# zilliztech/knowhere

Measured on NVIDIA H100. Metric: queries/sec at recall@10>=0.95, 10Mx128 f32 IVF_PQ, higher is better.
Workload: dtype f32

## Files before the change

knowhere_b200/csrc/kb2_index.cuh:

```cuda
#pragma once
#include <algorithm>
#include <functional>
#include <memory>
#include <mutex>
#include <vector>

#include "kb2_build.cuh"
#include "kb2_comm.h"
#include "kb2_fourcc.h"
#include "kb2_gemm_tc.cuh"
#include "kb2_ivf.cuh"
#include "kb2_ivfpq_tc.cuh"
#include "kb2_ivfflat_tc.cuh"
#include "kb2_json.h"
#include "kb2_large_k.cuh"

namespace kb2 {

constexpr int kMaxK = 1024;
constexpr int kMaxSortEntries = 8192;
constexpr int kMaxLargeK = 16384;
constexpr int64_t kLargeKScratch = 1ll << 30;

struct Counters {
// ... 1236 lines not shown
            KB2_CUDA_CHECK(cudaEventRecord(ev_join, side_stream));
            KB2_CUDA_CHECK(cudaStreamWaitEvent(st, ev_join, 0));
            side_pending = false;
        }
        mark("plan");
        pqtc::Params tp{};
        tp.metric = metric;
        tp.nq = (int)nq;
        tp.nprobe = nprobe;
        tp.queries = sp.queries;
        tp.qb16 = (const __nv_bfloat16*)s_qb16.p;
        tp.qnorm = s_qnorm.p;
        tp.n_items = items.n_items;
        tp.ticket = items.ticket;
        tp.item_list = items.list;
        tp.item_q0 = items.q0;
        tp.item_nq = items.nq;
        tp.pair_q = s_pair_q.p;
        tp.pair_base = s_pair_base.p;
        tp.bound = s_bound.p;
        tp.k_need = k_base;
        tp.margin_coef = (metric == KB2_METRIC_L2 ? 2.f : 1.f) * pqtc::kErrCoef * tc_rmax;
        tp.rmax = (metric == KB2_METRIC_L2) ? tc_rowmax : 0.f;
        tp.list_off = list_off.p;
        tp.list_len = list_len.p;
        tp.codes = (const uint4*)codes.p;
        tp.codes_plain = (const uint4*)tc_codes_plain.p;
        tp.npad = npad;
        tp.t1 = t1.p;
        tp.pqc = pqc.p;
        tp.pqc16 = (const uint4*)tc_pqc16.p;
        tp.bitset = sp.bitset;
        tp.rows = rows.p;
        const int n_logs = 2 * num_sms();
        const SurvivorLogs logs = alloc_logs(n_logs, (uint32_t)std::clamp<int64_t>(nq * 1024 / n_logs, 16384, 1 << 19));
        tp.log = logs.log;
        tp.log_cnt = logs.cnt;
        tp.log_cap = logs.cap;
        tp.qflag = s_cand_cnt.p + nq;
        tp.counters = d_counter.p;
        if (timing) KB2_CUDA_CHECK(cudaEventRecord(ev2, st));
        with_metric(metric, [&](auto m) {
            constexpr int MM = decltype(m)::value;
            if (tc_geom_18())
                launch<pqtc::ivfpq_tc_filter_kernel<MM, 1, 8>>(num_sms(), pqtc::THREADS, pqtc::TcCfg<1, 8>::SMEM_BYTES, st, tp);
            else
                launch<pqtc::ivfpq_tc_filter_kernel<MM, 3, 2>>(num_sms(), pqtc::THREADS, pqtc::TcCfg<3, 2>::SMEM_BYTES, st, tp);
        });
        if (timing) KB2_CUDA_CHECK(cudaEventRecord(ev3, st));
        KB2_CUDA_CHECK(cudaGetLastError());
#ifdef KB2_FILTER_STALLS
        pqtc::filter_stalls_print_kernel<<<1, 1, 0, st>>>(num_sms());
#endif
        mark("tc_filter");
        lm::scatter_survivors_kernel<<<dim3(16, n_logs), 256, 0, st>>>(logs.log, logs.cnt, logs.cap, s_cand.p, s_cand_cnt.p, kTcCandCap,
                                                                       tp.qflag, d_counter.p);
        const float* eval_lut = (tc_geom_18() && !dist) ? s_lut.p : nullptr;
        with_metric(metric, [&](auto m) {
            constexpr int MM = decltype(m)::value;
            if (tc_geom_18())
                pqtc::exact_eval_kernel<MM, 1, 8><<<(unsigned)nq, 128, 0, st>>>(sp.queries, pqc.p, eval_lut, s_bound.p, (const uint4*)codes.p,
                                                                               npad, t1.p, sp.bitset, rows.p, s_cand.p, s_cand_cnt.p,
                                                                               kTcCandCap, tp.qflag, logs.cnt + n_logs, k_base);
            else
                pqtc::exact_eval_kernel<MM, 3, 2><<<(unsigned)nq, 128, 0, st>>>(sp.queries, pqc.p, eval_lut, s_bound.p, (const uint4*)codes.p,
                                                                               npad, t1.p, sp.bitset, rows.p, s_cand.p, s_cand_cnt.p,
                                                                               kTcCandCap, tp.qflag, logs.cnt + n_logs, k_base);
        });
// ... 687 lines not shown
```

knowhere_b200/csrc/kb2_ivfpq_tc.cuh:

```cuda
#pragma once
#include <cuda_bf16.h>

#include <type_traits>
#include <utility>

#include "kb2_gemm_tc.cuh"
#include "kb2_ivf.cuh"
#include "kb2_listmajor.cuh"

namespace kb2 {
namespace pqtc {

using lm::TM;
constexpr int NQT = 256;
constexpr int THREADS = 512;
constexpr int GROUP_THREADS = 128;
constexpr int MAXW = 80;
constexpr int META_BYTES = 3 * NQT * 4;
template <int G, int DSUB>
struct TcCfg {
    static constexpr int M = 16 * G;
    static constexpr int KD = M * DSUB;
    static_assert(KD % 16 == 0 && (DSUB == 2 || DSUB == 4 || DSUB == 8), "unsupported PQ geometry");
    static constexpr int XCHUNK = KD / 8;
    static constexpr int KSTEPS = KD / 16 + 1;
    static constexpr int CHUNKS = 2 * KSTEPS;
    static constexpr int GRP_BYTES = CHUNKS * 128;
    static constexpr int TAB_BYTES = M * 256 * DSUB * 2;
    static constexpr int A_BYTES = (TM / 8) * GRP_BYTES, B_BYTES = (NQT / 8) * GRP_BYTES;
    static constexpr int OFF_TAB = 0;
    static constexpr int OFF_A = TAB_BYTES;
    static constexpr int OFF_B = OFF_A + 2 * A_BYTES;
    static constexpr int OFF_META = OFF_B + B_BYTES;
    static constexpr int OFF_BAR = OFF_META + 2 * META_BYTES;
    static constexpr size_t SMEM_BYTES = OFF_BAR + 256 + 128 ;
    static_assert(SMEM_BYTES <= 227 * 1024, "filter kernel shared memory");
};
constexpr int KD = 128;
constexpr float kErrCoef = 0.0085f;
constexpr float kAccCoef = 4e-5f;

struct Params {
    int metric;
    int nq, nprobe;
    const float* queries;
    const __nv_bfloat16* qb16;
    const float* qnorm;
    const int32_t* n_items;
    int32_t* ticket;
    const int32_t* item_list;
    const int32_t* item_q0;
    const int32_t* item_nq;
    const int32_t* pair_q;
    const float* pair_base;
    const float* bound;
    int k_need;
    float margin_coef;
    float rmax;
    const int64_t* list_off;
    const int32_t* list_len;
    const uint4* codes;
    const uint4* codes_plain;
    int64_t npad;
    const float* t1;
    const float* pqc;
    const uint4* pqc16;
    const uint8_t* bitset;
    const int32_t* rows;
    uint4* log;
    uint32_t* log_cnt;
    uint32_t log_cap;
    uint32_t* qflag;
    unsigned long long* counters;
};

template <typename F, int... I>
__device__ __forceinline__ void
static_for_impl(F&& f, std::integer_sequence<int, I...>) {
    (f(std::integral_constant<int, I>{}), ...);
}
template <int N, typename F>
__device__ __forceinline__ void
static_for(F&& f) {
    static_for_impl(f, std::make_integer_sequence<int, N>{});
}
template <int C0_, int W_>
struct BlockCols {
    static constexpr int C0 = C0_, W = W_;
};
template <int LO, int HI, typename F>
__device__ __forceinline__ void
dispatch_range(int n, F&& f) {
    if constexpr (LO == HI) {
        f(std::integral_constant<int, LO>{});
    } else {
        constexpr int MID = (LO + HI) / 2;
        if (n <= MID) dispatch_range<LO, MID>(n, f);
        else dispatch_range<MID + 1, HI>(n, f);
    }
}

__device__ __forceinline__ void
bar_sync_epi() {
    asm volatile("bar.sync 1, 256;" ::: "memory");
}
__device__ __forceinline__ uint64_t
make_desc_ns(uint32_t smem_addr, uint32_t grp_bytes) {
    uint64_t d = 0;
    d |= (uint64_t)((smem_addr & 0x3FFFFu) >> 4);
    d |= (uint64_t)(128 >> 4) << 16;
    d |= (uint64_t)(grp_bytes >> 4) << 32;
    return d;
}

#ifdef KB2_FILTER_STALLS
#define KB2_STALL_BEGIN(v) const long long v = clock64()
#define KB2_STALL_END(slot, v) stall[slot] += clock64() - (v)
constexpr int kStallMaxCtas = 1024, kStallSlots = 8;
__device__ unsigned long long g_filter_stalls[kStallMaxCtas][2][2][kStallSlots];
__global__ void
filter_stalls_print_kernel(int ctas) {
    for (int b = 0; b < min(ctas, kStallMaxCtas); b++) {
        printf("KB2STALL cta=%d", b);
        for (int r = 0; r < 2; r++) {
            printf(r == 0 ? " dec=" : " cons=");
            for (int i = 0; i < kStallSlots; i++)
                printf(i ? ",%llu" : "%llu", g_filter_stalls[b][r][0][i] + g_filter_stalls[b][r][1][i]);
        }
        printf("\n");
    }
}
#else
#define KB2_STALL_BEGIN(v)
#define KB2_STALL_END(slot, v)
#endif

__device__ __forceinline__ void
split3_bf16(float x, uint32_t& hi, uint32_t& mid, uint32_t& lo) {
    const __nv_bfloat16 h = __float2bfloat16_rn(x);
    hi = (uint32_t)__bfloat16_as_ushort(h);
    if (!(fabsf(x) < INFINITY)) { mid = 0u; lo = 0u; return; }
    const float r1 = x - __bfloat162float(h);
    const __nv_bfloat16 m = __float2bfloat16_rn(r1);
    const float r2 = r1 - __bfloat162float(m);
    mid = (uint32_t)__bfloat16_as_ushort(m);
    lo = (uint32_t)__bfloat16_as_ushort(__float2bfloat16_rn(r2));
}

template <int METRIC, int G, int DSUB>
__global__ void __launch_bounds__(THREADS, 1)
ivfpq_tc_filter_kernel(Params p) {
    using C = TcCfg<G, DSUB>;
    constexpr int KD = C::KD, XCHUNK = C::XCHUNK, KSTEPS = C::KSTEPS, GRP_BYTES = C::GRP_BYTES, TAB_BYTES = C::TAB_BYTES;
    constexpr int A_BYTES = C::A_BYTES, OFF_TAB = C::OFF_TAB, OFF_A = C::OFF_A, OFF_B = C::OFF_B, OFF_META = C::OFF_META,
                  OFF_BAR = C::OFF_BAR;
    extern __shared__ unsigned char smem_dyn[];
    const uint32_t raw = tc::smem_u32(smem_dyn);
    const uint32_t base = (raw + 127u) & ~127u;
    unsigned char* sm = smem_dyn + (base - raw);
    const uint32_t bars = base + OFF_BAR;
    auto bar_a_full = [&](int i) { return bars + 8u * i; };
    auto bar_a_empty = [&](int i) { return bars + 8u * (2 + i); };
    const uint32_t bar_b_full = bars + 8u * 8, bar_b_free = bars + 8u * 9;
    auto bar_meta_full = [&](int i) { return bars + 8u * (10 + i); };
    auto bar_meta_free = [&](int i) { return bars + 8u * (12 + i); };
    uint32_t* qcnt = (uint32_t*)(sm + OFF_BAR + 8 * 15);

    const int warp = __shfl_sync(0xffffffffu, (int)threadIdx.x >> 5, 0), lane = threadIdx.x & 31;
    const int n_items = *p.n_items;

    const lm::ItemRing<8> ring(sm + OFF_BAR + 144, p.ticket);
    ring.init();

    if (threadIdx.x == 0) {
        for (int i = 0; i < 2; i++) {
            tc::mbar_init(bar_a_full(i), GROUP_THREADS);
            tc::mbar_init(bar_a_empty(i), GROUP_THREADS);
            tc::mbar_init(bar_meta_full(i), 2 * GROUP_THREADS);
            tc::mbar_init(bar_meta_free(i), 2 * GROUP_THREADS);
        }
        tc::mbar_init(bar_b_full, 2 * GROUP_THREADS);
        tc::mbar_init(bar_b_free, 2 * GROUP_THREADS);
        qcnt[0] = qcnt[1] = qcnt[2] = qcnt[3] = 0;
        asm volatile("fence.mbarrier_init.release.cluster;" ::: "memory");
    }
#ifdef KB2_FILTER_STALLS
    long long stall[kStallSlots] = {0, 0, 0, 0, 0, 0, 0, 0};
    KB2_STALL_BEGIN(t_role);
#endif
    {
        uint4* tab = (uint4*)(sm + OFF_TAB);
        for (int i = threadIdx.x; i < TAB_BYTES / 16; i += THREADS) tab[i] = __ldg(p.pqc16 + i);
    }
    __syncthreads();
    const float inv_alpha = (METRIC == KB2_METRIC_L2) ? 0.5f : 1.f;

    if (warp < 8) {
        const int dt = threadIdx.x;
        const int dg = dt >> 7;
        const int tid = dt & 127;
        const uint4* tab = (const uint4*)(sm + OFF_TAB);
        auto write_meta = [&](int item, int it) {
            KB2_STALL_BEGIN(t_meta);
            const int par = it & 1;
            tc::mbar_wait(bar_meta_free(par), (((uint32_t)it >> 1) & 1u) ^ 1u);
            const int q0 = p.item_q0[item];
            const int nqi = p.item_nq[item];
            float* m_h = (float*)(sm + OFF_META + par * META_BYTES);
            float* m_base = m_h + NQT;
            int* m_q = (int*)(m_base + NQT);
            const int j = dt;
            float h = -INFINITY, bs = 0.f;
            int q = -1;
            if (j < nqi) {
                q = p.pair_q[q0 + j];
                bs = p.pair_base[q0 + j];
                const float bnd = p.bound[q];
                if (!(bnd < INFINITY)) {
                    p.qflag[q] = 1u;
                    if (p.counters) atomicAdd(p.counters + 6, 1ull << 32);
                } else {
                    const float margin = p.margin_coef * p.qnorm[q] * 1.01f + 1e-30f;
                    const float h0 = (bnd + margin - bs) * inv_alpha;
                    h = h0 + kAccCoef * (fabsf(h0) + p.rmax) + 1e-30f;
                }
            }
            m_h[j] = h;
            m_base[j] = bs;
            m_q[j] = q;
            tc::mbar_arrive(bar_meta_full(par));
            KB2_STALL_END(5, t_meta);
        };
        uint32_t g0 = 0;
        int it = 0;
        int item = ring.at_warp(0);
        if (item < n_items) write_meta(item, 0);
        for (; item < n_items; it++) {
            const int item_next = ring.at_warp(it + 1);
            const int l = p.item_list[item];
            const int nqi = p.item_nq[item];
            const int nmma = (nqi + 15) & ~15;
            const int len = p.list_len[l];
            const int64_t off = p.list_off[l];
            const int ntiles = (len + TM - 1) / TM;
            const int par = it & 1;
            const int t_first = (int)((dg - (int)(g0 & 1u)) & 1);
            uint4 w_next[G];
#pragma unroll
            for (int g = 0; g < G; g++) w_next[g] = make_uint4(0, 0, 0, 0);
            float t_next = 0.f;
            const uint4* code_src = (DSUB == 8) ? p.codes : p.codes_plain;
            if (t_first < ntiles && off + (int64_t)t_first * TM + tid < p.npad) {
#pragma unroll
                for (int g = 0; g < G; g++) w_next[g] = ldg_stream_u4(code_src + (int64_t)g * p.npad + off + (int64_t)t_first * TM + tid);
                if (METRIC == KB2_METRIC_L2) t_next = __ldg(p.t1 + off + (int64_t)t_first * TM + tid);
            }
            auto decode_tile = [&](int t) {
                KB2_STALL_BEGIN(t_dec);
                const uint32_t g = g0 + (uint32_t)t;
                uint4 w[G];
#pragma unroll
                for (int gg = 0; gg < G; gg++) w[gg] = w_next[gg];
                const float tv = t_next;
                {
                    const int64_t pn = off + (int64_t)(t + 2) * TM + tid;
                    if (t + 2 < ntiles && pn < p.npad) {
#pragma unroll
                        for (int gg = 0; gg < G; gg++) w_next[gg] = ldg_stream_u4(code_src + (int64_t)gg * p.npad + pn);
                        if (METRIC == KB2_METRIC_L2) t_next = __ldg(p.t1 + pn);
                    }
                }
                float r = INFINITY;
                if (t * TM + tid < len) r = (METRIC == KB2_METRIC_L2) ? 0.5f * tv : 0.f;
                uint32_t rh, rm, rl;
                split3_bf16(-r, rh, rm, rl);
                uint4 v[XCHUNK];
                if constexpr (DSUB == 8) {
#pragma unroll
                    for (int gg = 0; gg < G; gg++) {
                        const uint32_t ww[4] = {w[gg].x, w[gg].y, w[gg].z, w[gg].w};
#pragma unroll
                        for (int s = 0; s < 16; s++) {
                            const uint32_t byte = (ww[s >> 2] >> (8 * (s & 3))) & 255u;
                            v[gg * 16 + s] = tab[byte * (16 * G) + gg * 16 + ((s + tid) & 15)];
                        }
                    }
                } else {
                    constexpr int SPC = 8 / DSUB;
                    constexpr int WPS = DSUB / 2;
                    const uint32_t* tab32 = reinterpret_cast<const uint32_t*>(tab);
#pragma unroll
                    for (int c = 0; c < XCHUNK; c++) {
                        uint32_t u[4];
#pragma unroll
                        for (int j = 0; j < SPC; j++) {
                            const int m = c * SPC + j;
                            const uint4 wg = w[m >> 4];
                            const int b = m & 15;
                            const uint32_t word = (b < 4) ? wg.x : (b < 8) ? wg.y : (b < 12) ? wg.z : wg.w;
                            const uint32_t byte = (word >> (8 * (b & 3))) & 255u;
#pragma unroll
                            for (int x = 0; x < WPS; x++) u[j * WPS + x] = tab32[(m * 256 + byte) * WPS + x];
                        }
                        v[c] = make_uint4(u[0], u[1], u[2], u[3]);
                    }
                }
                KB2_STALL_BEGIN(t_ae);
                tc::mbar_wait(bar_a_empty(dg), ((g >> 1) & 1u) ^ 1u);
                KB2_STALL_END(1, t_ae);
                unsigned char* A = sm + OFF_A + dg * A_BYTES + (tid >> 3) * GRP_BYTES + (tid & 7) * 16;
#pragma unroll
                for (int c = 0; c < XCHUNK; c++) {
                    const int chunk = (DSUB == 8) ? (c & ~15) + ((c + tid) & 15) : c;
                    *reinterpret_cast<uint4*>(A + chunk * 128) = v[c];
                }
                *reinterpret_cast<uint4*>(A + XCHUNK * 128) = make_uint4(rh | (rm << 16), rl | (0x3F80u << 16), 0x3F803F80u, 0u);
                *reinterpret_cast<uint4*>(A + (XCHUNK + 1) * 128) = make_uint4(0u, 0u, 0u, 0u);
                tc::fence_proxy_async();
                tc::mbar_arrive(bar_a_full(dg));
                KB2_STALL_END(3, t_dec);
            };
            if (t_first < ntiles) decode_tile(t_first);
            KB2_STALL_BEGIN(t_b);
            asm volatile("bar.sync 2, 256;" ::: "memory");
            KB2_STALL_BEGIN(t_bf);
            tc::mbar_wait(bar_b_free, ((uint32_t)it & 1u) ^ 1u);
            KB2_STALL_END(2, t_bf);
            {
                const float* m_h = (const float*)(sm + OFF_META + par * META_BYTES);
                const int* m_q = (const int*)(m_h + 2 * NQT);
                const uint32_t Bs = base + OFF_B;
                unsigned char* B = sm + OFF_B;
                const int kc = tid >> 3;
                const int rsub = tid & 7;
                for (int blk = dg; blk < nmma / 8 && kc < XCHUNK; blk += 2) {
                    const int row = blk * 8 + rsub;
                    const int q = m_q[row];
                    const uint32_t dst = (uint32_t)(blk * GRP_BYTES + kc * 128 + rsub * 16);
                    if (q >= 0) {
                        const void* src = reinterpret_cast<const uint4*>(p.qb16 + (int64_t)q * KD) + kc;
                        asm volatile("cp.async.cg.shared.global [%0], [%1], 16;" ::"r"(Bs + dst), "l"(src) : "memory");
                    } else {
                        *reinterpret_cast<uint4*>(B + dst) = make_uint4(0, 0, 0, 0);
                    }
                }
                if (dt < nmma) {
                    uint32_t hh, hm, hl;
                    split3_bf16(m_h[dt], hh, hm, hl);
                    unsigned char* Bc = B + (dt >> 3) * GRP_BYTES + (dt & 7) * 16;
                    *reinterpret_cast<uint4*>(Bc + XCHUNK * 128) = make_uint4(0x3F803F80u, 0x3F80u | (hh << 16), hm | (hl << 16), 0u);
                    *reinterpret_cast<uint4*>(Bc + (XCHUNK + 1) * 128) = make_uint4(0u, 0u, 0u, 0u);
                }
                asm volatile("cp.async.wait_all;" ::: "memory");
            }
            tc::fence_proxy_async();
            tc::mbar_arrive(bar_b_full);
            KB2_STALL_END(4, t_b);
            if (item_next < n_items) write_meta(item_next, it + 1);
            for (int t = t_first + 2; t < ntiles; t += 2) decode_tile(t);
            g0 += (uint32_t)ntiles;
            item = item_next;
        }
    } else {
        const int et = threadIdx.x - 256;
        const int eg = et >> 7;
        const int e = et & 127;
        const int we = warp & 3;
        const uint32_t n_logs = 2u * gridDim.x;
        uint4* my_log = p.log + (size_t)(2 * blockIdx.x + eg) * p.log_cap;
        uint32_t* my_cursor = qcnt + eg;
        bool log_over = false;
        unsigned long long n_codes = 0;
        uint32_t g0 = 0;
        int it = 0;
        for (int item = ring.at_warp(0); item < n_items; item = ring.at_warp(++it)) {
            const int l = p.item_list[item];
            const int nqi = p.item_nq[item];
            const int ncls = __shfl_sync(0xffffffffu, (nqi + 15) >> 4, 0);
            const int len = p.list_len[l];
            const int64_t off = p.list_off[l];
            const int ntiles = (len + TM - 1) / TM;
            const int par = it & 1;
            KB2_STALL_BEGIN(t_mf);
            tc::mbar_wait(bar_meta_full(par), ((uint32_t)it >> 1) & 1u);
            KB2_STALL_END(1, t_mf);
            const float* m_base = (const float*)(sm + OFF_META + par * META_BYTES) + NQT;
            const int* m_q = (const int*)(m_base + NQT);
            if (et == 0) n_codes += (unsigned long long)len * (unsigned long long)nqi;
            const int t_first = (int)((eg - (int)(g0 & 1u)) & 1);
            KB2_STALL_BEGIN(t_bfull);
            tc::mbar_wait(bar_b_full, (uint32_t)it & 1u);
            KB2_STALL_END(2, t_bfull);
            const uint32_t a0 = base + OFF_A + eg * A_BYTES;
            const uint32_t b0 = base + OFF_B;
            const uint32_t la0 = (uint32_t)make_desc_ns(a0, GRP_BYTES), lb0 = (uint32_t)make_desc_ns(b0, GRP_BYTES);
            constexpr uint64_t desc_hi = (uint64_t)(GRP_BYTES >> 4) << 32;
            for (int t = t_first; t < ntiles; t += 2) {
                const uint32_t g = g0 + (uint32_t)t;
                KB2_STALL_BEGIN(t_af);
                tc::mbar_wait(bar_a_full(eg), (g >> 1) & 1u);
                KB2_STALL_END(3, t_af);
                auto issue = [&](auto& acc, int h, auto blk) {
                    using B = decltype(blk);
                    KB2_STALL_BEGIN(t_is);
                    uint32_t la = la0 + (uint32_t)(h * 8 * GRP_BYTES / 16), lb = lb0 + (uint32_t)(B::C0 / 8 * GRP_BYTES / 16);
                    if constexpr (G == 1) asm volatile("" : "+r"(la), "+r"(lb));
                    tc::fence_operand(acc);
                    tc::wgmma_fence();
#pragma unroll
                    for (int ks = 0; ks < KSTEPS; ks++)
                        tc::wgmma_bf16<B::W>(acc, desc_hi | (la + ks * 16u), desc_hi | (lb + ks * 16u), ks > 0 ? 1u : 0u);
                    tc::wgmma_commit();
                    tc::fence_operand(acc);
                    KB2_STALL_END(6, t_is);
                };
                uint64_t mh[2][2] = {{0ull, 0ull}, {0ull, 0ull}};
                auto test = [&](const auto& v, int h, auto blk) {
                    using B = decltype(blk);
                    constexpr int NBIT = B::W / 4, HALF = NBIT / 2;
                    KB2_STALL_BEGIN(t_te);
                    uint32_t n0l = 0u, n0h = 0u, n1l = 0u, n1h = 0u;
#pragma unroll
                    for (int i = HALF - 1; i >= 0; i--) {
                        const int x = 4 * (i >> 1) + (i & 1);
                        const int xh = 4 * ((i + HALF) >> 1) + ((i + HALF) & 1);
                        n0l = __funnelshift_l(__float_as_uint(v[x]), n0l, 1);
                        n0h = __funnelshift_l(__float_as_uint(v[xh]), n0h, 1);
                        n1l = __funnelshift_l(__float_as_uint(v[x + 2]), n1l, 1);
                        n1h = __funnelshift_l(__float_as_uint(v[xh + 2]), n1h, 1);
                    }
                    constexpr uint32_t mask = (1u << NBIT) - 1u;
                    const uint32_t m0 = ~((n0h << HALF) | n0l) & mask, m1 = ~((n1h << HALF) | n1l) & mask;
                    mh[h][0] |= (uint64_t)m0 << (B::C0 / 4);
                    mh[h][1] |= (uint64_t)m1 << (B::C0 / 4);
                    KB2_STALL_END(7, t_te);
                };
                auto flush = [&]() {
                    const uint32_t total =
                        (uint32_t)(__popcll(mh[0][0]) + __popcll(mh[0][1]) + __popcll(mh[1][0]) + __popcll(mh[1][1]));
                    if (total != 0u) {
                        uint32_t slot = atomicAdd(my_cursor, total);
#pragma unroll
                        for (int h = 0; h < 2; h++) {
#pragma unroll
                            for (int i = 0; i < 2; i++) {
                                const int rel = t * TM + h * 64 + we * 16 + (lane >> 2) + 8 * i;
                                uint64_t m = mh[h][i];
                                while (m) {
                                    const int bit = __ffsll((long long)m) - 1;
                                    m &= m - 1;
                                    const int col = 8 * (bit >> 1) + 2 * (lane & 3) + (bit & 1);
                                    if (slot < p.log_cap) {
                                        uint4 o;
                                        o.x = (uint32_t)m_q[col];
                                        o.y = (uint32_t)(off + rel);
                                        o.z = __float_as_uint(m_base[col]);
                                        o.w = 0u;
                                        my_log[slot] = o;
                                    } else {
                                        log_over = true;
                                    }
                                    slot++;
                                }
                            }
                        }
                    }
                };
                dispatch_range<1, NQT / 16>(ncls, [&](auto nc) {
                    constexpr int NC = decltype(nc)::value, NB = (16 * NC + MAXW - 1) / MAXW, NBT = 2 * NB;
                    constexpr int U = NC / NB, X = NC % NB;
                    auto blk = [](auto cc) {
                        constexpr int c = decltype(cc)::value;
                        return BlockCols<16 * (c * U + (c < X ? c : X)), 16 * (U + (c < X ? 1 : 0))>{};
                    };
                    float va[8 * (U + (X > 0 ? 1 : 0))], vb[8 * (U + (X > 0 ? 1 : 0))];
                    issue(va, 0, blk(std::integral_constant<int, 0>{}));
                    static_for<NBT>([&](auto bc) {
                        constexpr int b = decltype(bc)::value;
                        if constexpr (b + 1 < NBT) {
                            constexpr auto bn = blk(std::integral_constant<int, (b + 1) % NB>{});
                            if constexpr ((b + 1) & 1) issue(vb, (b + 1) / NB, bn);
                            else issue(va, (b + 1) / NB, bn);
                            KB2_STALL_BEGIN(t_w);
                            tc::wgmma_wait<1>();
                            KB2_STALL_END(4, t_w);
                        } else {
                            KB2_STALL_BEGIN(t_w);
                            tc::wgmma_wait<0>();
                            KB2_STALL_END(4, t_w);
                        }
                        constexpr auto bb = blk(std::integral_constant<int, b % NB>{});
                        if constexpr (b & 1) {
                            tc::fence_operand(vb);
                            test(vb, b / NB, bb);
                        } else {
                            tc::fence_operand(va);
                            test(va, b / NB, bb);
                        }
                    });
                });
                tc::mbar_arrive(bar_a_empty(eg));
                KB2_STALL_BEGIN(t_fl);
                flush();
                KB2_STALL_END(5, t_fl);
            }
            tc::mbar_arrive(bar_b_free);
            tc::mbar_arrive(bar_meta_free(par));
            g0 += (uint32_t)ntiles;
        }
        if (log_over) p.log_cnt[n_logs] = 1u;
        if (eg == 0) asm volatile("bar.sync 3, 128;" ::: "memory"); else asm volatile("bar.sync 4, 128;" ::: "memory");
        if (e == 0) {
            const uint32_t n = min(*my_cursor, p.log_cap);
            p.log_cnt[2 * blockIdx.x + eg] = n;
            if (p.counters) atomicAdd(p.counters + 2, (unsigned long long)n);
        }
        if (et == 0 && p.counters) atomicAdd(p.counters, n_codes);
    }
#ifdef KB2_FILTER_STALLS
    KB2_STALL_END(0, t_role);
    if ((threadIdx.x & 127) == 0 && blockIdx.x < kStallMaxCtas) {
        for (int i = 0; i < kStallSlots; i++)
            g_filter_stalls[blockIdx.x][warp >= 8][(threadIdx.x >> 7) & 1][i] = (unsigned long long)stall[i];
    }
#endif
}

__global__ void
prepare_queries_kernel(const float* __restrict__ q, int64_t nq, int d, __nv_bfloat16* __restrict__ qb16, float* __restrict__ qnorm) {
    const int64_t w = ((int64_t)blockIdx.x * blockDim.x + threadIdx.x) >> 5;
    const int lane = threadIdx.x & 31;
    if (w >= nq) return;
    float s = 0.f;
    for (int j = lane * 4; j < d; j += 128) {
        const float4 v = __ldg(reinterpret_cast<const float4*>(q + w * d + j));
        __nv_bfloat162 lo = __floats2bfloat162_rn(v.x, v.y), hi = __floats2bfloat162_rn(v.z, v.w);
        uint2 o;
        o.x = *reinterpret_cast<uint32_t*>(&lo);
        o.y = *reinterpret_cast<uint32_t*>(&hi);
        *reinterpret_cast<uint2*>(qb16 + w * d + j) = o;
        s += v.x * v.x + v.y * v.y + v.z * v.z + v.w * v.w;
    }
    s = warp_sum(s);
    if (lane == 0) qnorm[w] = sqrtf(s) * 1.0001f;
}

__global__ void __launch_bounds__(256)
prepare_tables_kernel(const float* __restrict__ pqc, int dsub, __nv_bfloat16* __restrict__ pqc16, float* __restrict__ maxn2) {
    const int m = blockIdx.x, j = threadIdx.x;
    const int M = gridDim.x;
    const float* c = pqc + ((size_t)m * 256 + j) * dsub;
    float n2 = 0.f;
    __nv_bfloat16* o = pqc16 + (dsub == 8 ? ((size_t)j * M + m) : ((size_t)m * 256 + j)) * dsub;
    for (int t = 0; t < dsub; t++) {
        n2 = fmaf(c[t], c[t], n2);
        o[t] = __float2bfloat16_rn(c[t]);
// ... 494 lines not shown
```

Measured before the change: 4.149 million.

## Restructure PQ filter kernel into four symmetric warpgroups with 64-row tiles

Replaces the producer/consumer warp specialization, where decoder warps filled A tiles and signalled consumer warpgroups through mbarriers, with four identical 128-thread warpgroups. Each warpgroup decodes its own 64-row tile into a private A buffer, runs WGMMA against the shared query B tile, and logs survivors. Named barriers replace the mbarrier handshakes, and survivor logs are doubled to one per warpgroup with smaller capacity. The aim is to remove cross-role waits and keep all warps busy. The cost is serialized decode and MMA inside each warpgroup and more barrier synchronization.

```diff
diff --git a/knowhere_b200/csrc/kb2_index.cuh b/knowhere_b200/csrc/kb2_index.cuh
--- a/knowhere_b200/csrc/kb2_index.cuh
+++ b/knowhere_b200/csrc/kb2_index.cuh
@@ -1292,8 +1292,8 @@
         tp.pqc16 = (const uint4*)tc_pqc16.p;
         tp.bitset = sp.bitset;
         tp.rows = rows.p;
-        const int n_logs = 2 * num_sms();
-        const SurvivorLogs logs = alloc_logs(n_logs, (uint32_t)std::clamp<int64_t>(nq * 1024 / n_logs, 16384, 1 << 19));
+        const int n_logs = 4 * num_sms();
+        const SurvivorLogs logs = alloc_logs(n_logs, (uint32_t)std::clamp<int64_t>(nq * 1024 / n_logs, 8192, 1 << 18));
         tp.log = logs.log;
         tp.log_cnt = logs.cnt;
         tp.log_cap = logs.cap;
diff --git a/knowhere_b200/csrc/kb2_ivfpq_tc.cuh b/knowhere_b200/csrc/kb2_ivfpq_tc.cuh
--- a/knowhere_b200/csrc/kb2_ivfpq_tc.cuh
+++ b/knowhere_b200/csrc/kb2_ivfpq_tc.cuh
@@ -11,7 +11,7 @@
 namespace kb2 {
 namespace pqtc {
 
-using lm::TM;
+constexpr int TT = 64;
 constexpr int NQT = 256;
 constexpr int THREADS = 512;
 constexpr int GROUP_THREADS = 128;
@@ -27,13 +27,14 @@
     static constexpr int CHUNKS = 2 * KSTEPS;
     static constexpr int GRP_BYTES = CHUNKS * 128;
     static constexpr int TAB_BYTES = M * 256 * DSUB * 2;
-    static constexpr int A_BYTES = (TM / 8) * GRP_BYTES, B_BYTES = (NQT / 8) * GRP_BYTES;
+    static constexpr int A_BYTES = (TT / 8) * GRP_BYTES, B_BYTES = (NQT / 8) * GRP_BYTES;
     static constexpr int OFF_TAB = 0;
     static constexpr int OFF_A = TAB_BYTES;
-    static constexpr int OFF_B = OFF_A + 2 * A_BYTES;
+    static constexpr int OFF_B = OFF_A + 4 * A_BYTES;
     static constexpr int OFF_META = OFF_B + B_BYTES;
-    static constexpr int OFF_BAR = OFF_META + 2 * META_BYTES;
-    static constexpr size_t SMEM_BYTES = OFF_BAR + 256 + 128 ;
+    static constexpr int OFF_CTL = OFF_META + 2 * META_BYTES;
+    static constexpr size_t SMEM_BYTES = OFF_CTL + 128 + 128 ;
+    static_assert(16 + lm::ItemRing<8>::BYTES <= 128, "filter kernel control words");
     static_assert(SMEM_BYTES <= 227 * 1024, "filter kernel shared memory");
 };
 constexpr int KD = 128;
@@ -88,6 +89,20 @@
 struct BlockCols {
     static constexpr int C0 = C0_, W = W_;
 };
+template <int NC, int NB>
+__host__ __device__ constexpr int
+block_units(int c) {
+    constexpr int U = NC / NB, X = NC % NB;
+    const bool wide = (NB == 3 && X == 1) ? c == 1 : (NB == 3 && X == 2) ? c != 1 : c < X;
+    return U + (wide ? 1 : 0);
+}
+template <int NC, int NB>
+__host__ __device__ constexpr int
+block_start(int c) {
+    int s = 0;
+    for (int i = 0; i < c; i++) s += block_units<NC, NB>(i);
+    return s;
+}
 template <int LO, int HI, typename F>
 __device__ __forceinline__ void
 dispatch_range(int n, F&& f) {
@@ -100,10 +115,6 @@
     }
 }
 
-__device__ __forceinline__ void
-bar_sync_epi() {
-    asm volatile("bar.sync 1, 256;" ::: "memory");
-}
 __device__ __forceinline__ uint64_t
 make_desc_ns(uint32_t smem_addr, uint32_t grp_bytes) {
     uint64_t d = 0;
@@ -116,16 +127,15 @@
 #ifdef KB2_FILTER_STALLS
 #define KB2_STALL_BEGIN(v) const long long v = clock64()
 #define KB2_STALL_END(slot, v) stall[slot] += clock64() - (v)
-constexpr int kStallMaxCtas = 1024, kStallSlots = 8;
-__device__ unsigned long long g_filter_stalls[kStallMaxCtas][2][2][kStallSlots];
+constexpr int kStallMaxCtas = 1024, kStallSlots = 8, kStallGroups = 4;
+__device__ unsigned long long g_filter_stalls[kStallMaxCtas][kStallGroups][kStallSlots];
 __global__ void
 filter_stalls_print_kernel(int ctas) {
     for (int b = 0; b < min(ctas, kStallMaxCtas); b++) {
         printf("KB2STALL cta=%d", b);
-        for (int r = 0; r < 2; r++) {
-            printf(r == 0 ? " dec=" : " cons=");
-            for (int i = 0; i < kStallSlots; i++)
-                printf(i ? ",%llu" : "%llu", g_filter_stalls[b][r][0][i] + g_filter_stalls[b][r][1][i]);
+        for (int w = 0; w < kStallGroups; w++) {
+            printf(" wg%d=", w);
+            for (int i = 0; i < kStallSlots; i++) printf(i ? ",%llu" : "%llu", g_filter_stalls[b][w][i]);
         }
         printf("\n");
     }
@@ -147,46 +157,43 @@
     lo = (uint32_t)__bfloat16_as_ushort(__float2bfloat16_rn(r2));
 }
 
+__device__ __forceinline__ void
+bar_sync_cta(int id) {
+    asm volatile("bar.sync %0, %1;" ::"r"(id), "n"(THREADS) : "memory");
+}
+__device__ __forceinline__ void
+bar_sync_wg(int wg) {
+    asm volatile("bar.sync %0, %1;" ::"r"(3 + wg), "n"(GROUP_THREADS) : "memory");
+}
+
 template <int METRIC, int G, int DSUB>
 __global__ void __launch_bounds__(THREADS, 1)
 ivfpq_tc_filter_kernel(Params p) {
     using C = TcCfg<G, DSUB>;
     constexpr int KD = C::KD, XCHUNK = C::XCHUNK, KSTEPS = C::KSTEPS, GRP_BYTES = C::GRP_BYTES, TAB_BYTES = C::TAB_BYTES;
     constexpr int A_BYTES = C::A_BYTES, OFF_TAB = C::OFF_TAB, OFF_A = C::OFF_A, OFF_B = C::OFF_B, OFF_META = C::OFF_META,
-                  OFF_BAR = C::OFF_BAR;
+                  OFF_CTL = C::OFF_CTL;
+    constexpr int HALF = XCHUNK / 2, SPC = 8 / DSUB, WPS = DSUB / 2;
     extern __shared__ unsigned char smem_dyn[];
     const uint32_t raw = tc::smem_u32(smem_dyn);
     const uint32_t base = (raw + 127u) & ~127u;
     unsigned char* sm = smem_dyn + (base - raw);
-    const uint32_t bars = base + OFF_BAR;
-    auto bar_a_full = [&](int i) { return bars + 8u * i; };
-    auto bar_a_empty = [&](int i) { return bars + 8u * (2 + i); };
-    const uint32_t bar_b_full = bars + 8u * 8, bar_b_free = bars + 8u * 9;
-    auto bar_meta_full = [&](int i) { return bars + 8u * (10 + i); };
-    auto bar_meta_free = [&](int i) { return bars + 8u * (12 + i); };
-    uint32_t* qcnt = (uint32_t*)(sm + OFF_BAR + 8 * 15);
+    uint32_t* qcnt = (uint32_t*)(sm + OFF_CTL);
 
     const int warp = __shfl_sync(0xffffffffu, (int)threadIdx.x >> 5, 0), lane = threadIdx.x & 31;
+    const int wg = warp >> 2;
+    const int e = threadIdx.x & 127;
+    const int we = warp & 3;
+    const int row = we * 16 + (lane & 15);
+    const int hh = lane >> 4;
     const int n_items = *p.n_items;
 
-    const lm::ItemRing<8> ring(sm + OFF_BAR + 144, p.ticket);
+    const lm::ItemRing<8> ring(sm + OFF_CTL + 16, p.ticket);
     ring.init();
-
-    if (threadIdx.x == 0) {
-        for (int i = 0; i < 2; i++) {
-            tc::mbar_init(bar_a_full(i), GROUP_THREADS);
-            tc::mbar_init(bar_a_empty(i), GROUP_THREADS);
-            tc::mbar_init(bar_meta_full(i), 2 * GROUP_THREADS);
-            tc::mbar_init(bar_meta_free(i), 2 * GROUP_THREADS);
-        }
-        tc::mbar_init(bar_b_full, 2 * GROUP_THREADS);
-        tc::mbar_init(bar_b_free, 2 * GROUP_THREADS);
-        qcnt[0] = qcnt[1] = qcnt[2] = qcnt[3] = 0;
-        asm volatile("fence.mbarrier_init.release.cluster;" ::: "memory");
-    }
+    if (threadIdx.x < 4) qcnt[threadIdx.x] = 0u;
 #ifdef KB2_FILTER_STALLS
     long long stall[kStallSlots] = {0, 0, 0, 0, 0, 0, 0, 0};
-    KB2_STALL_BEGIN(t_role);
+    KB2_STALL_BEGIN(t_all);
 #endif
     {
         uint4* tab = (uint4*)(sm + OFF_TAB);
@@ -194,334 +201,303 @@
     }
     __syncthreads();
     const float inv_alpha = (METRIC == KB2_METRIC_L2) ? 0.5f : 1.f;
-
-    if (warp < 8) {
-        const int dt = threadIdx.x;
-        const int dg = dt >> 7;
-        const int tid = dt & 127;
-        const uint4* tab = (const uint4*)(sm + OFF_TAB);
-        auto write_meta = [&](int item, int it) {
-            KB2_STALL_BEGIN(t_meta);
-            const int par = it & 1;
-            tc::mbar_wait(bar_meta_free(par), (((uint32_t)it >> 1) & 1u) ^ 1u);
-            const int q0 = p.item_q0[item];
-            const int nqi = p.item_nq[item];
-            float* m_h = (float*)(sm + OFF_META + par * META_BYTES);
-            float* m_base = m_h + NQT;
-            int* m_q = (int*)(m_base + NQT);
-            const int j = dt;
-            float h = -INFINITY, bs = 0.f;
-            int q = -1;
-            if (j < nqi) {
-                q = p.pair_q[q0 + j];
-                bs = p.pair_base[q0 + j];
-                const float bnd = p.bound[q];
-                if (!(bnd < INFINITY)) {
-                    p.qflag[q] = 1u;
+    const uint4* tab = (const uint4*)(sm + OFF_TAB);
+    const uint4* code_src = (DSUB == 8) ? p.codes : p.codes_plain;
+
+    auto write_meta = [&](int item, int it) {
+        const int q0 = p.item_q0[item];
+        const int nqi = p.item_nq[item];
+        float* m_h = (float*)(sm + OFF_META + (it & 1) * META_BYTES);
+        float* m_base = m_h + NQT;
+        int* m_q = (int*)(m_base + NQT);
+        int q[2];
+        float bs[2], bnd[2], qn[2];
+#pragma unroll
+        for (int i = 0; i < 2; i++) {
+            const int j = e + 128 * i;
+            q[i] = (j < nqi) ? p.pair_q[q0 + j] : -1;
+            bs[i] = (j < nqi) ? p.pair_base[q0 + j] : 0.f;
+        }
+#pragma unroll
+        for (int i = 0; i < 2; i++) {
+            bnd[i] = (q[i] >= 0) ? p.bound[q[i]] : INFINITY;
+            qn[i] = (q[i] >= 0) ? p.qnorm[q[i]] : 0.f;
+        }
+#pragma unroll
+        for (int i = 0; i < 2; i++) {
+            const int j = e + 128 * i;
+            float h = -INFINITY;
+            if (q[i] >= 0) {
+                if (!(bnd[i] < INFINITY)) {
+                    p.qflag[q[i]] = 1u;
                     if (p.counters) atomicAdd(p.counters + 6, 1ull << 32);
                 } else {
-                    const float margin = p.margin_coef * p.qnorm[q] * 1.01f + 1e-30f;
-                    const float h0 = (bnd + margin - bs) * inv_alpha;
+                    const float margin = p.margin_coef * qn[i] * 1.01f + 1e-30f;
+                    const float h0 = (bnd[i] + margin - bs[i]) * inv_alpha;
                     h = h0 + kAccCoef * (fabsf(h0) + p.rmax) + 1e-30f;
                 }
             }
             m_h[j] = h;
-            m_base[j] = bs;
-            m_q[j] = q;
-            tc::mbar_arrive(bar_meta_full(par));
-            KB2_STALL_END(5, t_meta);
+            m_base[j] = bs[i];
+            m_q[j] = q[i];
+        }
+    };
+
+    uint2 wn[G];
+#pragma unroll
+    for (int k = 0; k < G; k++) wn[k] = make_uint2(0u, 0u);
+    float tn = 0.f;
+    auto load = [&](int64_t tile_pos) {
+        const int64_t pos = tile_pos + row;
+        if (pos < p.npad) {
+#pragma unroll
+            for (int k = 0; k < G; k++) {
+                const int u = G * hh + k;
+                wn[k] = ldg_stream_u2(reinterpret_cast<const uint2*>(code_src + (int64_t)(u >> 1) * p.npad + pos) + (u & 1));
+            }
+            if (METRIC == KB2_METRIC_L2 && hh == 0) tn = __ldg(p.t1 + pos);
+        }
+    };
+
+    bool log_over = false;
+    uint32_t* my_cursor = qcnt + wg;
+    const uint32_t a0 = base + OFF_A + wg * A_BYTES;
+    unsigned char* A = sm + OFF_A + wg * A_BYTES + (row >> 3) * GRP_BYTES + (row & 7) * 16;
+
+    uint32_t g0 = 0;
+    int it = 0;
+    int item = ring.at_warp(0);
+    if (item < n_items) {
+        if (wg == 0) write_meta(item, 0);
+        const int l = p.item_list[item];
+        const int tf = wg;
+        if (tf < (p.list_len[l] + TT - 1) / TT) load(p.list_off[l] + (int64_t)tf * TT);
+    }
+    for (; item < n_items; it++) {
+        const int item_next = ring.at_warp(it + 1);
+        const int l = p.item_list[item];
+        const int nqi = p.item_nq[item];
+        const int nu = (nqi + 15) >> 4;
+        const int ncls = __shfl_sync(0xffffffffu, nu == 5 ? 6 : nu, 0);
+        const int len = p.list_len[l];
+        const int64_t off = p.list_off[l];
+        const int ntiles = (len + TT - 1) / TT;
+        const int t_first = (int)(((uint32_t)wg - g0) & 3u);
+        int64_t pf_next = -1;
+        if (item_next < n_items) {
+            const int ln = p.item_list[item_next];
+            const int tf_n = (int)(((uint32_t)wg - (g0 + (uint32_t)ntiles)) & 3u);
+            if (tf_n < (p.list_len[ln] + TT - 1) / TT) pf_next = p.list_off[ln] + (int64_t)tf_n * TT;
+        }
+        if (threadIdx.x == 0 && p.counters) atomicAdd(p.counters, (unsigned long long)len * (unsigned long long)nqi);
+
+        auto decode = [&](int t) {
+            KB2_STALL_BEGIN(t_dec);
+            uint32_t wd[2 * G];
+#pragma unroll
+            for (int k = 0; k < G; k++) { wd[2 * k] = wn[k].x; wd[2 * k + 1] = wn[k].y; }
+            const float tv = tn;
+            if (t + 4 < ntiles) load(off + (int64_t)(t + 4) * TT);
+            else if (pf_next >= 0) load(pf_next);
+            float r = INFINITY;
+            if (t * TT + row < len) r = (METRIC == KB2_METRIC_L2) ? 0.5f * tv : 0.f;
+            uint32_t rh, rm, rl;
+            split3_bf16(-r, rh, rm, rl);
+            uint4 v[HALF];
+#pragma unroll
+            for (int i = 0; i < HALF; i++) {
+                if constexpr (DSUB == 8) {
+                    const uint32_t byte = (wd[i >> 2] >> (8 * (i & 3))) & 255u;
+                    const int c = HALF * hh + i;
+                    v[i] = tab[byte * (16 * G) + (c & ~15) + ((c + row) & 15)];
+                } else {
+                    const uint32_t* tab32 = reinterpret_cast<const uint32_t*>(tab);
+                    uint32_t u[4];
+#pragma unroll
+                    for (int j = 0; j < SPC; j++) {
+                        const int b = i * SPC + j;
+                        const uint32_t byte = (wd[b >> 2] >> (8 * (b & 3))) & 255u;
+                        const int m = 8 * G * hh + b;
+#pragma unroll
+                        for (int x = 0; x < WPS; x++) u[j * WPS + x] = tab32[(m * 256 + byte) * WPS + x];
+                    }
+                    v[i] = make_uint4(u[0], u[1], u[2], u[3]);
+                }
+            }
+            KB2_STALL_END(1, t_dec);
+            KB2_STALL_BEGIN(t_b1);
+            bar_sync_wg(wg);
+            KB2_STALL_END(2, t_b1);
+            KB2_STALL_BEGIN(t_st);
+#pragma unroll
+            for (int i = 0; i < HALF; i++) {
+                const int c = HALF * hh + i;
+                const int chunk = (DSUB == 8) ? (c & ~15) + ((c + row) & 15) : c;
+                *reinterpret_cast<uint4*>(A + chunk * 128) = v[i];
+            }
+            *reinterpret_cast<uint4*>(A + (XCHUNK + hh) * 128) =
+                hh ? make_uint4(0u, 0u, 0u, 0u) : make_uint4(rh | (rm << 16), rl | (0x3F80u << 16), 0x3F803F80u, 0u);
+            tc::fence_proxy_async();
+            KB2_STALL_END(1, t_st);
+            KB2_STALL_BEGIN(t_b2);
+            bar_sync_wg(wg);
+            KB2_STALL_END(2, t_b2);
         };
-        uint32_t g0 = 0;
-        int it = 0;
-        int item = ring.at_warp(0);
-        if (item < n_items) write_meta(item, 0);
-        for (; item < n_items; it++) {
-            const int item_next = ring.at_warp(it + 1);
-            const int l = p.item_list[item];
-            const int nqi = p.item_nq[item];
-            const int nmma = (nqi + 15) & ~15;
-            const int len = p.list_len[l];
-            const int64_t off = p.list_off[l];
-            const int ntiles = (len + TM - 1) / TM;
-            const int par = it & 1;
-            const int t_first = (int)((dg - (int)(g0 & 1u)) & 1);
-            uint4 w_next[G];
-#pragma unroll
-            for (int g = 0; g < G; g++) w_next[g] = make_uint4(0, 0, 0, 0);
-            float t_next = 0.f;
-            const uint4* code_src = (DSUB == 8) ? p.codes : p.codes_plain;
-            if (t_first < ntiles && off + (int64_t)t_first * TM + tid < p.npad) {
-#pragma unroll
-                for (int g = 0; g < G; g++) w_next[g] = ldg_stream_u4(code_src + (int64_t)g * p.npad + off + (int64_t)t_first * TM + tid);
-                if (METRIC == KB2_METRIC_L2) t_next = __ldg(p.t1 + off + (int64_t)t_first * TM + tid);
-            }
-            auto decode_tile = [&](int t) {
-                KB2_STALL_BEGIN(t_dec);
-                const uint32_t g = g0 + (uint32_t)t;
-                uint4 w[G];
-#pragma unroll
-                for (int gg = 0; gg < G; gg++) w[gg] = w_next[gg];
-                const float tv = t_next;
-                {
-                    const int64_t pn = off + (int64_t)(t + 2) * TM + tid;
-                    if (t + 2 < ntiles && pn < p.npad) {
-#pragma unroll
-                        for (int gg = 0; gg < G; gg++) w_next[gg] = ldg_stream_u4(code_src + (int64_t)gg * p.npad + pn);
-                        if (METRIC == KB2_METRIC_L2) t_next = __ldg(p.t1 + pn);
+
+        if (t_first < ntiles) decode(t_first);
+        else if (pf_next >= 0) load(pf_next);
+        {
+            KB2_STALL_BEGIN(t_b);
+            bar_sync_cta(1);
+            const float* m_h = (const float*)(sm + OFF_META + (it & 1) * META_BYTES);
+            const int* m_q = (const int*)(m_h + 2 * NQT);
+            const uint32_t Bs = base + OFF_B;
+            unsigned char* B = sm + OFF_B;
+            const int nmma = 16 * ncls;
+            for (int i = threadIdx.x; i < nmma * XCHUNK; i += THREADS) {
+                const int blk = i / (8 * XCHUNK), rem = i - blk * (8 * XCHUNK);
+                const int kc = rem >> 3, rsub = rem & 7;
+                const int q = m_q[blk * 8 + rsub];
+                const uint32_t dst = (uint32_t)(blk * GRP_BYTES + kc * 128 + rsub * 16);
+                if (q >= 0) {
+                    const void* src = reinterpret_cast<const uint4*>(p.qb16 + (int64_t)q * KD) + kc;
+                    asm volatile("cp.async.cg.shared.global [%0], [%1], 16;" ::"r"(Bs + dst), "l"(src) : "memory");
+                } else {
+                    *reinterpret_cast<uint4*>(B + dst) = make_uint4(0, 0, 0, 0);
+                }
+            }
+            if ((int)threadIdx.x < nmma) {
+                uint32_t hh_, hm, hl;
+                split3_bf16(m_h[threadIdx.x], hh_, hm, hl);
+                unsigned char* Bc = B + (threadIdx.x >> 3) * GRP_BYTES + (threadIdx.x & 7) * 16;
+                *reinterpret_cast<uint4*>(Bc + XCHUNK * 128) = make_uint4(0x3F803F80u, 0x3F80u | (hh_ << 16), hm | (hl << 16), 0u);
+                *reinterpret_cast<uint4*>(Bc + (XCHUNK + 1) * 128) = make_uint4(0u, 0u, 0u, 0u);
+            }
+            asm volatile("cp.async.wait_all;" ::: "memory");
+            tc::fence_proxy_async();
+            bar_sync_cta(2);
+            if (wg == (it & 3) && item_next < n_items) write_meta(item_next, it + 1);
+            KB2_STALL_END(7, t_b);
+        }
+
+        const uint32_t la0 = (uint32_t)make_desc_ns(a0, GRP_BYTES), lb0 = (uint32_t)make_desc_ns(base + OFF_B, GRP_BYTES);
+        constexpr uint64_t desc_hi = (uint64_t)(GRP_BYTES >> 4) << 32;
+        for (int t = t_first; t < ntiles; t += 4) {
+            if (t != t_first) decode(t);
+            auto issue = [&](auto& acc, auto blk) {
+                using Bk = decltype(blk);
+                KB2_STALL_BEGIN(t_is);
+                uint32_t la = la0, lb = lb0 + (uint32_t)(Bk::C0 / 8 * GRP_BYTES / 16);
+                if constexpr (G == 1) asm volatile("" : "+r"(la), "+r"(lb));
+                tc::fence_operand(acc);
+                tc::wgmma_fence();
+#pragma unroll
+                for (int ks = 0; ks < KSTEPS; ks++)
+                    tc::wgmma_bf16<Bk::W>(acc, desc_hi | (la + ks * 16u), desc_hi | (lb + ks * 16u), ks > 0 ? 1u : 0u);
+                tc::wgmma_commit();
+                tc::fence_operand(acc);
+                KB2_STALL_END(3, t_is);
+            };
+            uint64_t mh[2] = {0ull, 0ull};
+            auto test = [&](const auto& v, auto blk) {
+                using Bk = decltype(blk);
+                constexpr int NBIT = Bk::W / 4, HB = NBIT / 2;
+                KB2_STALL_BEGIN(t_te);
+                uint32_t n0l = 0u, n0h = 0u, n1l = 0u, n1h = 0u;
+#pragma unroll
+                for (int i = HB - 1; i >= 0; i--) {
+                    const int x = 4 * (i >> 1) + (i & 1);
+                    const int xh = 4 * ((i + HB) >> 1) + ((i + HB) & 1);
+                    n0l = __funnelshift_l(__float_as_uint(v[x]), n0l, 1);
+                    n0h = __funnelshift_l(__float_as_uint(v[xh]), n0h, 1);
+                    n1l = __funnelshift_l(__float_as_uint(v[x + 2]), n1l, 1);
+                    n1h = __funnelshift_l(__float_as_uint(v[xh + 2]), n1h, 1);
+                }
+                constexpr uint32_t mask = (1u << NBIT) - 1u;
+                const uint32_t m0 = ~((n0h << HB) | n0l) & mask, m1 = ~((n1h << HB) | n1l) & mask;
+                mh[0] |= (uint64_t)m0 << (Bk::C0 / 4);
+                mh[1] |= (uint64_t)m1 << (Bk::C0 / 4);
+                KB2_STALL_END(5, t_te);
+            };
+            auto body = [&](auto nc) {
+                constexpr int NC = decltype(nc)::value, NB = (16 * NC + MAXW - 1) / MAXW;
+                auto blk = [](auto cc) {
+                    constexpr int c = decltype(cc)::value;
+                    return BlockCols<16 * block_start<NC, NB>(c), 16 * block_units<NC, NB>(c)>{};
+                };
+                float va[8 * block_units<NC, NB>(0)], vb[8 * block_units<NC, NB>(NB > 1 ? 1 : 0)];
+                issue(va, blk(std::integral_constant<int, 0>{}));
+                static_for<NB>([&](auto bc) {
+                    constexpr int b = decltype(bc)::value;
+                    if constexpr (b + 1 < NB) {
+                        constexpr auto bn = blk(std::integral_constant<int, b + 1>{});
+                        if constexpr ((b + 1) & 1) issue(vb, bn);
+                        else issue(va, bn);
+                        KB2_STALL_BEGIN(t_w);
+                        tc::wgmma_wait<1>();
+                        KB2_STALL_END(4, t_w);
+                    } else {
+                        KB2_STALL_BEGIN(t_w);
+                        tc::wgmma_wait<0>();
+                        KB2_STALL_END(4, t_w);
+                    }
+                    constexpr auto bb = blk(std::integral_constant<int, b>{});
+                    if constexpr (b & 1) {
+                        tc::fence_operand(vb);
+                        test(vb, bb);
+                    } else {
+                        tc::fence_operand(va);
+                        test(va, bb);
+                    }
+                });
+            };
+            if (ncls <= 4) dispatch_range<1, 4>(ncls, body);
+            else dispatch_range<6, NQT / 16>(ncls, body);
+            KB2_STALL_BEGIN(t_fl);
+            const uint32_t total = (uint32_t)(__popcll(mh[0]) + __popcll(mh[1]));
+            if (total != 0u) {
+                uint4* my_log = p.log + (size_t)(4 * blockIdx.x + wg) * p.log_cap;
+                const float* m_base = (const float*)(sm + OFF_META + (it & 1) * META_BYTES) + NQT;
+                const int* m_q = (const int*)(m_base + NQT);
+                uint32_t slot = atomicAdd(my_cursor, total);
+#pragma unroll
+                for (int i = 0; i < 2; i++) {
+                    const int rel = t * TT + we * 16 + (lane >> 2) + 8 * i;
+                    uint64_t m = mh[i];
+                    while (m) {
+                        const int bit = __ffsll((long long)m) - 1;
+                        m &= m - 1;
+                        const int col = 8 * (bit >> 1) + 2 * (lane & 3) + (bit & 1);
+                        if (slot < p.log_cap) {
+                            uint4 o;
+                            o.x = (uint32_t)m_q[col];
+                            o.y = (uint32_t)(off + rel);
+                            o.z = __float_as_uint(m_base[col]);
+                            o.w = 0u;
+                            my_log[slot] = o;
+                        } else {
+                            log_over = true;
+                        }
+                        slot++;
                     }
                 }
-                float r = INFINITY;
-                if (t * TM + tid < len) r = (METRIC == KB2_METRIC_L2) ? 0.5f * tv : 0.f;
-                uint32_t rh, rm, rl;
-                split3_bf16(-r, rh, rm, rl);
-                uint4 v[XCHUNK];
-                if constexpr (DSUB == 8) {
-#pragma unroll
-                    for (int gg = 0; gg < G; gg++) {
-                        const uint32_t ww[4] = {w[gg].x, w[gg].y, w[gg].z, w[gg].w};
-#pragma unroll
-                        for (int s = 0; s < 16; s++) {
-                            const uint32_t byte = (ww[s >> 2] >> (8 * (s & 3))) & 255u;
-                            v[gg * 16 + s] = tab[byte * (16 * G) + gg * 16 + ((s + tid) & 15)];
-                        }
-                    }
-                } else {
-                    constexpr int SPC = 8 / DSUB;
-                    constexpr int WPS = DSUB / 2;
-                    const uint32_t* tab32 = reinterpret_cast<const uint32_t*>(tab);
-#pragma unroll
-                    for (int c = 0; c < XCHUNK; c++) {
-                        uint32_t u[4];
-#pragma unroll
-                        for (int j = 0; j < SPC; j++) {
-                            const int m = c * SPC + j;
-                            const uint4 wg = w[m >> 4];
-                            const int b = m & 15;
-                            const uint32_t word = (b < 4) ? wg.x : (b < 8) ? wg.y : (b < 12) ? wg.z : wg.w;
-                            const uint32_t byte = (word >> (8 * (b & 3))) & 255u;
-#pragma unroll
-                            for (int x = 0; x < WPS; x++) u[j * WPS + x] = tab32[(m * 256 + byte) * WPS + x];
-                        }
-                        v[c] = make_uint4(u[0], u[1], u[2], u[3]);
-                    }
-                }
-                KB2_STALL_BEGIN(t_ae);
-                tc::mbar_wait(bar_a_empty(dg), ((g >> 1) & 1u) ^ 1u);
-                KB2_STALL_END(1, t_ae);
-                unsigned char* A = sm + OFF_A + dg * A_BYTES + (tid >> 3) * GRP_BYTES + (tid & 7) * 16;
-#pragma unroll
-                for (int c = 0; c < XCHUNK; c++) {
-                    const int chunk = (DSUB == 8) ? (c & ~15) + ((c + tid) & 15) : c;
-                    *reinterpret_cast<uint4*>(A + chunk * 128) = v[c];
-                }
-                *reinterpret_cast<uint4*>(A + XCHUNK * 128) = make_uint4(rh | (rm << 16), rl | (0x3F80u << 16), 0x3F803F80u, 0u);
-                *reinterpret_cast<uint4*>(A + (XCHUNK + 1) * 128) = make_uint4(0u, 0u, 0u, 0u);
-                tc::fence_proxy_async();
-                tc::mbar_arrive(bar_a_full(dg));
-                KB2_STALL_END(3, t_dec);
-            };
-            if (t_first < ntiles) decode_tile(t_first);
-            KB2_STALL_BEGIN(t_b);
-            asm volatile("bar.sync 2, 256;" ::: "memory");
-            KB2_STALL_BEGIN(t_bf);
-            tc::mbar_wait(bar_b_free, ((uint32_t)it & 1u) ^ 1u);
-            KB2_STALL_END(2, t_bf);
-            {
-                const float* m_h = (const float*)(sm + OFF_META + par * META_BYTES);
-                const int* m_q = (const int*)(m_h + 2 * NQT);
-                const uint32_t Bs = base + OFF_B;
-                unsigned char* B = sm + OFF_B;
-                const int kc = tid >> 3;
-                const int rsub = tid & 7;
-                for (int blk = dg; blk < nmma / 8 && kc < XCHUNK; blk += 2) {
-                    const int row = blk * 8 + rsub;
-                    const int q = m_q[row];
-                    const uint32_t dst = (uint32_t)(blk * GRP_BYTES + kc * 128 + rsub * 16);
-                    if (q >= 0) {
-                        const void* src = reinterpret_cast<const uint4*>(p.qb16 + (int64_t)q * KD) + kc;
-                        asm volatile("cp.async.cg.shared.global [%0], [%1], 16;" ::"r"(Bs + dst), "l"(src) : "memory");
-                    } else {
-                        *reinterpret_cast<uint4*>(B + dst) = make_uint4(0, 0, 0, 0);
-                    }
-                }
-                if (dt < nmma) {
-                    uint32_t hh, hm, hl;
-                    split3_bf16(m_h[dt], hh, hm, hl);
-                    unsigned char* Bc = B + (dt >> 3) * GRP_BYTES + (dt & 7) * 16;
-                    *reinterpret_cast<uint4*>(Bc + XCHUNK * 128) = make_uint4(0x3F803F80u, 0x3F80u | (hh << 16), hm | (hl << 16), 0u);
-                    *reinterpret_cast<uint4*>(Bc + (XCHUNK + 1) * 128) = make_uint4(0u, 0u, 0u, 0u);
-                }
-                asm volatile("cp.async.wait_all;" ::: "memory");
-            }
-            tc::fence_proxy_async();
-            tc::mbar_arrive(bar_b_full);
-            KB2_STALL_END(4, t_b);
-            if (item_next < n_items) write_meta(item_next, it + 1);
-            for (int t = t_first + 2; t < ntiles; t += 2) decode_tile(t);
-            g0 += (uint32_t)ntiles;
-            item = item_next;
-        }
-    } else {
-        const int et = threadIdx.x - 256;
-        const int eg = et >> 7;
-        const int e = et & 127;
-        const int we = warp & 3;
-        const uint32_t n_logs = 2u * gridDim.x;
-        uint4* my_log = p.log + (size_t)(2 * blockIdx.x + eg) * p.log_cap;
-        uint32_t* my_cursor = qcnt + eg;
-        bool log_over = false;
-        unsigned long long n_codes = 0;
-        uint32_t g0 = 0;
-        int it = 0;
-        for (int item = ring.at_warp(0); item < n_items; item = ring.at_warp(++it)) {
-            const int l = p.item_list[item];
-            const int nqi = p.item_nq[item];
-            const int ncls = __shfl_sync(0xffffffffu, (nqi + 15) >> 4, 0);
-            const int len = p.list_len[l];
-            const int64_t off = p.list_off[l];
-            const int ntiles = (len + TM - 1) / TM;
-            const int par = it & 1;
-            KB2_STALL_BEGIN(t_mf);
-            tc::mbar_wait(bar_meta_full(par), ((uint32_t)it >> 1) & 1u);
-            KB2_STALL_END(1, t_mf);
-            const float* m_base = (const float*)(sm + OFF_META + par * META_BYTES) + NQT;
-            const int* m_q = (const int*)(m_base + NQT);
-            if (et == 0) n_codes += (unsigned long long)len * (unsigned long long)nqi;
-            const int t_first = (int)((eg - (int)(g0 & 1u)) & 1);
-            KB2_STALL_BEGIN(t_bfull);
-            tc::mbar_wait(bar_b_full, (uint32_t)it & 1u);
-            KB2_STALL_END(2, t_bfull);
-            const uint32_t a0 = base + OFF_A + eg * A_BYTES;
-            const uint32_t b0 = base + OFF_B;
-            const uint32_t la0 = (uint32_t)make_desc_ns(a0, GRP_BYTES), lb0 = (uint32_t)make_desc_ns(b0, GRP_BYTES);
-            constexpr uint64_t desc_hi = (uint64_t)(GRP_BYTES >> 4) << 32;
-            for (int t = t_first; t < ntiles; t += 2) {
-                const uint32_t g = g0 + (uint32_t)t;
-                KB2_STALL_BEGIN(t_af);
-                tc::mbar_wait(bar_a_full(eg), (g >> 1) & 1u);
-                KB2_STALL_END(3, t_af);
-                auto issue = [&](auto& acc, int h, auto blk) {
-                    using B = decltype(blk);
-                    KB2_STALL_BEGIN(t_is);
-                    uint32_t la = la0 + (uint32_t)(h * 8 * GRP_BYTES / 16), lb = lb0 + (uint32_t)(B::C0 / 8 * GRP_BYTES / 16);
-                    if constexpr (G == 1) asm volatile("" : "+r"(la), "+r"(lb));
-                    tc::fence_operand(acc);
-                    tc::wgmma_fence();
-#pragma unroll
-                    for (int ks = 0; ks < KSTEPS; ks++)
-                        tc::wgmma_bf16<B::W>(acc, desc_hi | (la + ks * 16u), desc_hi | (lb + ks * 16u), ks > 0 ? 1u : 0u);
-                    tc::wgmma_commit();
-                    tc::fence_operand(acc);
-                    KB2_STALL_END(6, t_is);
-                };
-                uint64_t mh[2][2] = {{0ull, 0ull}, {0ull, 0ull}};
-                auto test = [&](const auto& v, int h, auto blk) {
-                    using B = decltype(blk);
-                    constexpr int NBIT = B::W / 4, HALF = NBIT / 2;
-                    KB2_STALL_BEGIN(t_te);
-                    uint32_t n0l = 0u, n0h = 0u, n1l = 0u, n1h = 0u;
-#pragma unroll
-                    for (int i = HALF - 1; i >= 0; i--) {
-                        const int x = 4 * (i >> 1) + (i & 1);
-                        const int xh = 4 * ((i + HALF) >> 1) + ((i + HALF) & 1);
-                        n0l = __funnelshift_l(__float_as_uint(v[x]), n0l, 1);
-                        n0h = __funnelshift_l(__float_as_uint(v[xh]), n0h, 1);
-                        n1l = __funnelshift_l(__float_as_uint(v[x + 2]), n1l, 1);
-                        n1h = __funnelshift_l(__float_as_uint(v[xh + 2]), n1h, 1);
-                    }
-                    constexpr uint32_t mask = (1u << NBIT) - 1u;
-                    const uint32_t m0 = ~((n0h << HALF) | n0l) & mask, m1 = ~((n1h << HALF) | n1l) & mask;
-                    mh[h][0] |= (uint64_t)m0 << (B::C0 / 4);
-                    mh[h][1] |= (uint64_t)m1 << (B::C0 / 4);
-                    KB2_STALL_END(7, t_te);
-                };
-                auto flush = [&]() {
-                    const uint32_t total =
-                        (uint32_t)(__popcll(mh[0][0]) + __popcll(mh[0][1]) + __popcll(mh[1][0]) + __popcll(mh[1][1]));
-                    if (total != 0u) {
-                        uint32_t slot = atomicAdd(my_cursor, total);
-#pragma unroll
-                        for (int h = 0; h < 2; h++) {
-#pragma unroll
-                            for (int i = 0; i < 2; i++) {
-                                const int rel = t * TM + h * 64 + we * 16 + (lane >> 2) + 8 * i;
-                                uint64_t m = mh[h][i];
-                                while (m) {
-                                    const int bit = __ffsll((long long)m) - 1;
-                                    m &= m - 1;
-                                    const int col = 8 * (bit >> 1) + 2 * (lane & 3) + (bit & 1);
-                                    if (slot < p.log_cap) {
-                                        uint4 o;
-                                        o.x = (uint32_t)m_q[col];
-                                        o.y = (uint32_t)(off + rel);
-                                        o.z = __float_as_uint(m_base[col]);
-                                        o.w = 0u;
-                                        my_log[slot] = o;
-                                    } else {
-                                        log_over = true;
-                                    }
-                                    slot++;
-                                }
-                            }
-                        }
-                    }
-                };
-                dispatch_range<1, NQT / 16>(ncls, [&](auto nc) {
-                    constexpr int NC = decltype(nc)::value, NB = (16 * NC + MAXW - 1) / MAXW, NBT = 2 * NB;
-                    constexpr int U = NC / NB, X = NC % NB;
-                    auto blk = [](auto cc) {
-                        constexpr int c = decltype(cc)::value;
-                        return BlockCols<16 * (c * U + (c < X ? c : X)), 16 * (U + (c < X ? 1 : 0))>{};
-                    };
-                    float va[8 * (U + (X > 0 ? 1 : 0))], vb[8 * (U + (X > 0 ? 1 : 0))];
-                    issue(va, 0, blk(std::integral_constant<int, 0>{}));
-                    static_for<NBT>([&](auto bc) {
-                        constexpr int b = decltype(bc)::value;
-                        if constexpr (b + 1 < NBT) {
-                            constexpr auto bn = blk(std::integral_constant<int, (b + 1) % NB>{});
-                            if constexpr ((b + 1) & 1) issue(vb, (b + 1) / NB, bn);
-                            else issue(va, (b + 1) / NB, bn);
-                            KB2_STALL_BEGIN(t_w);
-                            tc::wgmma_wait<1>();
-                            KB2_STALL_END(4, t_w);
-                        } else {
-                            KB2_STALL_BEGIN(t_w);
-                            tc::wgmma_wait<0>();
-                            KB2_STALL_END(4, t_w);
-                        }
-                        constexpr auto bb = blk(std::integral_constant<int, b % NB>{});
-                        if constexpr (b & 1) {
-                            tc::fence_operand(vb);
-                            test(vb, b / NB, bb);
-                        } else {
-                            tc::fence_operand(va);
-                            test(va, b / NB, bb);
-                        }
-                    });
-                });
-                tc::mbar_arrive(bar_a_empty(eg));
-                KB2_STALL_BEGIN(t_fl);
-                flush();
-                KB2_STALL_END(5, t_fl);
-            }
-            tc::mbar_arrive(bar_b_free);
-            tc::mbar_arrive(bar_meta_free(par));
-            g0 += (uint32_t)ntiles;
-        }
-        if (log_over) p.log_cnt[n_logs] = 1u;
-        if (eg == 0) asm volatile("bar.sync 3, 128;" ::: "memory"); else asm volatile("bar.sync 4, 128;" ::: "memory");
-        if (e == 0) {
-            const uint32_t n = min(*my_cursor, p.log_cap);
-            p.log_cnt[2 * blockIdx.x + eg] = n;
-            if (p.counters) atomicAdd(p.counters + 2, (unsigned long long)n);
-        }
-        if (et == 0 && p.counters) atomicAdd(p.counters, n_codes);
+            }
+            KB2_STALL_END(6, t_fl);
+        }
+        g0 += (uint32_t)ntiles;
+        item = item_next;
+    }
+    if (log_over) p.log_cnt[4 * gridDim.x] = 1u;
+    bar_sync_wg(wg);
+    if (e == 0) {
+        const uint32_t n = min(*my_cursor, p.log_cap);
+        p.log_cnt[4 * blockIdx.x + wg] = n;
+        if (p.counters) atomicAdd(p.counters + 2, (unsigned long long)n);
     }
 #ifdef KB2_FILTER_STALLS
-    KB2_STALL_END(0, t_role);
-    if ((threadIdx.x & 127) == 0 && blockIdx.x < kStallMaxCtas) {
-        for (int i = 0; i < kStallSlots; i++)
-            g_filter_stalls[blockIdx.x][warp >= 8][(threadIdx.x >> 7) & 1][i] = (unsigned long long)stall[i];
+    KB2_STALL_END(0, t_all);
+    if (e == 0 && blockIdx.x < kStallMaxCtas) {
+        for (int i = 0; i < kStallSlots; i++) g_filter_stalls[blockIdx.x][wg][i] = (unsigned long long)stall[i];
     }
 #endif
 }
```

New measurement: 4.206 million (median of 6 runs). No clear change (+1.4%).
